# Oneflow-Inc/libai

Measured on AMD Instinct MI355X. Metric: tokens/sec (whole node), GPT-2 345M 3D-parallel at 1/2/4/8 MI355X, higher is better.
Workload: dtype bf16; 1 GPU; model=gpt2-345m (nl24 h1024 nah16 seq1024), global_batch=48, seq_len=1024, parallelism=dp1

## Files before the change

### libai_amd/csrc/kernels/adamw.hip

```cpp
#include "common.h"
#include "launchers.h"

namespace {

constexpr int CHUNK = 1 << 16;

struct AdamChunkDesc {
  int64_t param;
  int64_t master;
  int64_t grad;
  int64_t m;
  int64_t v;
  int64_t n;
};

template <class E>
__global__ void adamw_kernel(const AdamChunkDesc* __restrict__ chunks, float lr,
                             float beta1, float beta2, float eps, float wd,
                             float bc1, float bc2,
                             float grad_scale) {
  const AdamChunkDesc c = chunks[blockIdx.x];
  const int64_t n = c.n;
  typename E::T* p16 = (typename E::T*)c.param;
  float* master = (float*)c.master;
  const typename E::T* g = (const typename E::T*)c.grad;
  float* m = (float*)c.m;
  float* v = (float*)c.v;
  const float inv_bc1 = 1.0f / bc1, inv_bc2 = 1.0f / bc2;

  for (int64_t i = threadIdx.x; i < n; i += blockDim.x) {
    float gv = E::to_f(g[i]) * grad_scale;
    float pv = master[i];
    float mv = m[i] = beta1 * m[i] + (1.0f - beta1) * gv;
    float vv = v[i] = beta2 * v[i] + (1.0f - beta2) * gv * gv;
    float mhat = mv * inv_bc1;
    float vhat = vv * inv_bc2;
    pv -= lr * (mhat / (sqrtf(vhat) + eps) + wd * pv);
    master[i] = pv;
    if (p16) p16[i] = E::from_f(pv);
  }
}

struct NormChunkDesc {
  int64_t ptr;
  int64_t n;
};

template <class E>
__global__ void l2norm_sq_kernel(const NormChunkDesc* __restrict__ chunks,
                                 float* __restrict__ out) {
  __shared__ float red[16];
  const NormChunkDesc c = chunks[blockIdx.x];
  const typename E::T* x = (const typename E::T*)c.ptr;
  float s = 0.f;
  for (int64_t i = threadIdx.x; i < c.n; i += blockDim.x) {
    float v = E::to_f(x[i]);
    s += v * v;
  }
  s = block_reduce(s, red, SumOp(), 0.f);
  if (threadIdx.x == 0) atomicAdd(out, s);
}

}

extern "C" int adamw_chunk_elems() { return CHUNK; }

#define ADAMW_LAUNCHERS(SUFF, ETYPE)                                                   \
  extern "C" void adamw_step_##SUFF(const void* chunks, int nchunks, float lr,         \
                                    float beta1, float beta2, float eps, float wd,     \
                                    float bc1, float bc2, float grad_scale,            \
                                    hipStream_t stream) {                              \
    adamw_kernel<ETYPE><<<dim3(nchunks), dim3(256), 0, stream>>>(                      \
        (const AdamChunkDesc*)chunks, lr, beta1, beta2, eps, wd, bc1, bc2,             \
        grad_scale);                                                                   \
  }                                                                                    \
  extern "C" void l2norm_sq_##SUFF(const void* chunks, int nchunks, float* out,        \
                                   hipStream_t stream) {                               \
    l2norm_sq_kernel<ETYPE><<<dim3(nchunks), dim3(256), 0, stream>>>(                  \
        (const NormChunkDesc*)chunks, out);                                            \
  }

ADAMW_LAUNCHERS(bf16, BF16Elem)
ADAMW_LAUNCHERS(f32, F32Elem)
```

### libai_amd/csrc/kernels/common.h

```cpp
#pragma once
#include <hip/hip_runtime.h>
#include <stdint.h>

#include <type_traits>

#define WAVE 64

__device__ __forceinline__ float bf2f(uint16_t h) {
  union {
    uint32_t u;
    float f;
  } v;
  v.u = ((uint32_t)h) << 16;
  return v.f;
}

__device__ __forceinline__ uint16_t f2bf(float f) {
  union {
    float f;
    uint32_t u;
  } v;
  v.f = f;
  uint32_t lsb = (v.u >> 16) & 1u;
  uint32_t rounded = v.u + 0x7fffu + lsb;
  if ((v.u & 0x7f800000u) == 0x7f800000u) rounded = v.u;
  return (uint16_t)(rounded >> 16);
}

typedef uint16_t u16x8 __attribute__((ext_vector_type(8)));
typedef uint16_t u16x4 __attribute__((ext_vector_type(4)));
typedef float f32x4 __attribute__((ext_vector_type(4)));

struct BF16Elem {
  using T = uint16_t;
  static constexpr int VEC = 8;
  using VecT = u16x8;
  static __device__ __forceinline__ float to_f(T x) { return bf2f(x); }
  static __device__ __forceinline__ T from_f(float x) { return f2bf(x); }
};

struct F32Elem {
  using T = float;
  static constexpr int VEC = 4;
  using VecT = f32x4;
  static __device__ __forceinline__ float to_f(T x) { return x; }
  static __device__ __forceinline__ T from_f(float x) { return x; }
};

__device__ __forceinline__ float wave_reduce_sum(float v) {
#pragma unroll
  for (int off = WAVE / 2; off > 0; off >>= 1) v += __shfl_xor(v, off, WAVE);
  return v;
}

__device__ __forceinline__ float wave_reduce_max(float v) {
#pragma unroll
  for (int off = WAVE / 2; off > 0; off >>= 1) v = fmaxf(v, __shfl_xor(v, off, WAVE));
  return v;
}

template <typename Op>
__device__ __forceinline__ float block_reduce(float v, float* lds, Op op, float ident) {
  const int lane = threadIdx.x & (WAVE - 1);
  const int wid = threadIdx.x / WAVE;
  const int nw = (blockDim.x + WAVE - 1) / WAVE;
#pragma unroll
  for (int off = WAVE / 2; off > 0; off >>= 1) v = op(v, __shfl_xor(v, off, WAVE));
  if (lane == 0) lds[wid] = v;
  __syncthreads();
  v = (threadIdx.x < nw) ? lds[threadIdx.x] : ident;
  if (wid == 0) {
#pragma unroll
    for (int off = WAVE / 2; off > 0; off >>= 1) v = op(v, __shfl_xor(v, off, WAVE));
    if (lane == 0) lds[0] = v;
  }
  __syncthreads();
  v = lds[0];
  __syncthreads();
  return v;
}

struct SumOp {
  __device__ float operator()(float a, float b) const { return a + b; }
};
struct MaxOp {
  __device__ float operator()(float a, float b) const { return fmaxf(a, b); }
};

__device__ __forceinline__ void philox_round(uint32_t& c0, uint32_t& c1, uint32_t& c2,
                                             uint32_t& c3, uint32_t k0, uint32_t k1) {
  const uint32_t M0 = 0xD2511F53u, M1 = 0xCD9E8D57u;
  uint32_t h0 = __umulhi(M0, c0), l0 = M0 * c0;
  uint32_t h1 = __umulhi(M1, c2), l1 = M1 * c2;
  uint32_t n0 = h1 ^ c1 ^ k0;
  uint32_t n1 = l1;
  uint32_t n2 = h0 ^ c3 ^ k1;
  uint32_t n3 = l0;
  c0 = n0;
  c1 = n1;
  c2 = n2;
  c3 = n3;
}

__device__ __forceinline__ void philox4(uint64_t seed, uint64_t ctr, uint32_t out[4]) {
  uint32_t k0 = (uint32_t)seed, k1 = (uint32_t)(seed >> 32);
  uint32_t c0 = (uint32_t)ctr, c1 = (uint32_t)(ctr >> 32), c2 = 0x9E3779B9u, c3 = 0xBB67AE85u;
#pragma unroll
  for (int i = 0; i < 10; ++i) {
    philox_round(c0, c1, c2, c3, k0, k1);
    k0 += 0x9E3779B9u;
    k1 += 0xBB67AE85u;
  }
  out[0] = c0;
  out[1] = c1;
  out[2] = c2;
  out[3] = c3;
}

__device__ __forceinline__ float u32_to_uniform(uint32_t x) {
  return (x >> 8) * (1.0f / 16777216.0f);
}

#define RND_HASH_LO_MUL 0x9E3779B9u
#define RND_HASH_HI_MUL 0x85EBCA6Bu

__device__ __forceinline__ uint32_t rnd_hash_mix(uint32_t h) {
  h ^= h >> 16;
  h *= 0x7FEB352Du;
  h ^= h >> 15;
  h *= 0x846CA68Bu;
  h ^= h >> 16;
  return h;
}

__device__ __forceinline__ uint32_t rnd_hash2(uint64_t seed, uint32_t lo,
                                               uint32_t hi) {
  return rnd_hash_mix((uint32_t)seed ^ (lo * RND_HASH_LO_MUL) ^
                      (hi * RND_HASH_HI_MUL) ^ (uint32_t)(seed >> 32));
}

__device__ __forceinline__ uint32_t rnd_hash(uint64_t seed, uint64_t idx) {
  return rnd_hash2(seed, (uint32_t)idx, (uint32_t)(idx >> 32));
}

__device__ __forceinline__ uint32_t drop_threshold_u8(float p) {
  float t = p * 256.0f + 0.5f;
  return t >= 255.f ? 255u : (uint32_t)t;
}

__device__ __forceinline__ uint32_t drop_threshold_u32(float p) {
  double t = (double)p * 4294967296.0;
  return (t >= 4294967295.0) ? 0xFFFFFFFFu : (uint32_t)t;
}

__device__ __forceinline__ float fast_erff(float x) {
  const float a1 = 0.254829592f, a2 = -0.284496736f, a3 = 1.421413741f;
  const float a4 = -1.453152027f, a5 = 1.061405429f, p = 0.3275911f;
  float ax = fabsf(x);
  float t = 1.0f / fmaf(p, ax, 1.0f);
  float poly = t * fmaf(t, fmaf(t, fmaf(t, fmaf(t, a5, a4), a3), a2), a1);
  float y = 1.0f - poly * __expf(-ax * ax);
  return copysignf(y, x);
}

__device__ __forceinline__ float gelu_erf(float x) {
  return 0.5f * x * (1.0f + fast_erff(x * 0.70710678118654752440f));
}

__device__ __forceinline__ float gelu_erf_grad(float x) {
  const float kInvSqrt2 = 0.70710678118654752440f;
  const float kInvSqrt2Pi = 0.3989422804014327f;
  float cdf = 0.5f * (1.0f + fast_erff(x * kInvSqrt2));
  float pdf = kInvSqrt2Pi * __expf(-0.5f * x * x);
  return cdf + x * pdf;
}

#define CDIV(a, b) (((a) + (b)-1) / (b))

enum class FlashVariant : int { kPlain, kAlibi, kWindow, kRelBias, kDocs };

inline FlashVariant flash_variant(const float* alibi_slopes, int window,
                                  const float* rel_bias, const int* doc_start) {
  if (alibi_slopes != nullptr) return FlashVariant::kAlibi;
  if (window > 0) return FlashVariant::kWindow;
  if (rel_bias != nullptr) return FlashVariant::kRelBias;
  if (doc_start != nullptr) return FlashVariant::kDocs;
  return FlashVariant::kPlain;
}

template <class F>
void flash_dispatch(int D, FlashVariant v, F&& f) {
  auto on_d = [&](auto d) {
#define FLASH_VARIANT_CASE(NAME)                                             \
  case FlashVariant::NAME:                                                   \
    f(d, std::integral_constant<FlashVariant, FlashVariant::NAME>{});        \
    break;
    switch (v) {
      FLASH_VARIANT_CASE(kPlain)
      FLASH_VARIANT_CASE(kAlibi)
      FLASH_VARIANT_CASE(kWindow)
      FLASH_VARIANT_CASE(kRelBias)
      FLASH_VARIANT_CASE(kDocs)
    }
#undef FLASH_VARIANT_CASE
  };
  if (D == 64) on_d(std::integral_constant<int, 64>{});
  else if (D == 128) on_d(std::integral_constant<int, 128>{});
}
```

### libai_amd/csrc/kernels/fused_bias.hip

```cpp
#include "common.h"
#include "launchers.h"

namespace {

template <class E, bool GRAD>
__global__ void bias_gelu_kernel(const typename E::T* __restrict__ x,
                                 const typename E::T* __restrict__ b,
                                 const typename E::T* __restrict__ dy,
                                 typename E::T* __restrict__ out,
                                 float* __restrict__ db_partial, int64_t n,
                                 int W) {
  using VecT = typename E::VecT;
  constexpr int V = E::VEC;
  const int wvec = W / V;
  const int64_t R = n / W;
  const int cv = blockIdx.x * blockDim.x + threadIdx.x;
  if (cv >= wvec) return;
  VecT vb;
  if (b) vb = ((const VecT*)b)[cv];
  float db[GRAD ? V : 1] = {0.f};
  for (int64_t r = blockIdx.y; r < R; r += gridDim.y) {
    const int64_t i = r * wvec + cv;
    VecT vx = ((const VecT*)x)[i];
    VecT o;
    if (GRAD) {
      VecT vdy = ((const VecT*)dy)[i];
#pragma unroll
      for (int j = 0; j < V; ++j) {
        float xv = E::to_f(vx[j]) + (b ? E::to_f(vb[j]) : 0.f);
        float g = E::to_f(vdy[j]) * gelu_erf_grad(xv);
        o[j] = E::from_f(g);
        db[j] += g;
      }
    } else {
#pragma unroll
      for (int j = 0; j < V; ++j) {
        float xv = E::to_f(vx[j]) + (b ? E::to_f(vb[j]) : 0.f);
        o[j] = E::from_f(gelu_erf(xv));
      }
    }
    ((VecT*)out)[i] = o;
  }
  if (GRAD && db_partial != nullptr) {
#pragma unroll
    for (int j = 0; j < V; ++j)
      db_partial[(int64_t)blockIdx.y * W + cv * V + j] = db[j];
  }
}

template <class E, bool GRAD>
__global__ void bias_dropout_res_kernel(const typename E::T* __restrict__ x,
                                        const typename E::T* __restrict__ b,
                                        const typename E::T* __restrict__ res,
                                        typename E::T* __restrict__ out,
                                        float* __restrict__ db_partial, int64_t n,
                                        int W, float p, uint64_t seed) {
  using VecT = typename E::VecT;
  constexpr int V = E::VEC;
  const int wvec = W / V;
  const int64_t R = n / W;
  const float scale = 1.0f / (1.0f - p);
  const uint32_t thr8 = drop_threshold_u8(p);
  const int cv = blockIdx.x * blockDim.x + threadIdx.x;
  if (cv >= wvec) return;
  VecT vb;
  if (b) vb = ((const VecT*)b)[cv];
  float db[GRAD ? V : 1] = {0.f};
  for (int64_t r = blockIdx.y; r < R; r += gridDim.y) {
    const int64_t i = r * wvec + cv;
    VecT vx = ((const VecT*)x)[i];
    float keep[V];
    if (p > 0.f) {
#pragma unroll
      for (int q = 0; q < V / 4; ++q) {
        const uint64_t idx = (uint64_t)i * (V / 4) + q;
        const uint32_t h = rnd_hash(seed, idx);
#pragma unroll
        for (int j = 0; j < 4; ++j)
          keep[q * 4 + j] = (((h >> (j * 8)) & 0xFFu) >= thr8) ? scale : 0.f;
      }
    } else {
#pragma unroll
      for (int j = 0; j < V; ++j) keep[j] = 1.f;
    }
    VecT o;
    if (GRAD) {
#pragma unroll
      for (int j = 0; j < V; ++j) {
        float g = E::to_f(vx[j]) * keep[j];
        o[j] = E::from_f(g);
        db[j] += g;
      }
    } else {
      VecT vr;
      if (res) vr = ((const VecT*)res)[i];
#pragma unroll
      for (int j = 0; j < V; ++j) {
        float v = (E::to_f(vx[j]) + (b ? E::to_f(vb[j]) : 0.f)) * keep[j];
        o[j] = E::from_f(v + (res ? E::to_f(vr[j]) : 0.f));
      }
    }
    ((VecT*)out)[i] = o;
  }
  if (GRAD && db_partial != nullptr) {
#pragma unroll
    for (int j = 0; j < V; ++j)
      db_partial[(int64_t)blockIdx.y * W + cv * V + j] = db[j];
  }
}

template <class E>
__global__ void colsum_partial_kernel(const typename E::T* __restrict__ in,
                                      float* __restrict__ partial, int64_t R, int W) {
  using VecT = typename E::VecT;
  constexpr int V = E::VEC;
  const int wv = W / V;
  const int jv = blockIdx.x * blockDim.x + threadIdx.x;
  if (jv >= wv) return;
  const int P = gridDim.y;
  float s[V];
#pragma unroll
  for (int j = 0; j < V; ++j) s[j] = 0.f;
  for (int64_t r = blockIdx.y; r < R; r += P) {
    VecT v = ((const VecT*)(in + r * W))[jv];
#pragma unroll
    for (int j = 0; j < V; ++j) s[j] += E::to_f(v[j]);
  }
#pragma unroll
  for (int j = 0; j < V; ++j) partial[(int64_t)blockIdx.y * W + jv * V + j] = s[j];
}

template <class E>
__global__ void colsum_partial_scalar_kernel(const typename E::T* __restrict__ in,
                                             float* __restrict__ partial, int64_t R,
                                             int W) {
  const int j = blockIdx.x * blockDim.x + threadIdx.x;
  if (j >= W) return;
  const int P = gridDim.y;
  float s = 0.f;
  for (int64_t r = blockIdx.y; r < R; r += P) s += E::to_f(in[r * W + j]);
  partial[(int64_t)blockIdx.y * W + j] = s;
}

inline int64_t ew_grid(int64_t nvec) {
  int64_t g = CDIV(nvec, 256);
  return g < 2048 ? g : 2048;
}

inline dim3 col_grid(int64_t n, int W, int V, int* block_out) {
  const int wvec = W / V;
  const int block = wvec < 256 ? wvec : 256;
  const int gx = (int)CDIV(wvec, block);
  int64_t rows = n / W;
  int64_t gy = 4096 / gx;
  if (gy > rows) gy = rows;
  if (gy < 1) gy = 1;
  *block_out = block;
  return dim3(gx, (uint32_t)gy);
}

}

extern "C" int bias_col_grid_rows(int64_t n, int W, int V) {
  int blk;
  dim3 g = col_grid(n, W, V, &blk);
  return (int)g.y;
}

#define BIAS_LAUNCHERS(SUFF, ETYPE)                                                      \
  extern "C" void bias_gelu_fwd_##SUFF(const void* x, const void* b, void* y, int64_t n, \
                                       int W, hipStream_t stream) {                      \
    int blk;                                                                             \
    dim3 g = col_grid(n, W, ETYPE::VEC, &blk);                                           \
    bias_gelu_kernel<ETYPE, false><<<g, dim3(blk), 0, stream>>>(                         \
        (const ETYPE::T*)x, (const ETYPE::T*)b, nullptr, (ETYPE::T*)y, nullptr, n,       \
        W);                                                                              \
  }                                                                                      \
  extern "C" void bias_gelu_bwd_##SUFF(const void* x, const void* b, const void* dy,     \
                                       void* dx, float* db_partial, int64_t n, int W,    \
                                       hipStream_t stream) {                             \
    int blk;                                                                             \
    dim3 g = col_grid(n, W, ETYPE::VEC, &blk);                                           \
    bias_gelu_kernel<ETYPE, true><<<g, dim3(blk), 0, stream>>>(                          \
        (const ETYPE::T*)x, (const ETYPE::T*)b, (const ETYPE::T*)dy, (ETYPE::T*)dx,      \
        db_partial, n, W);                                                               \
  }                                                                                      \
  extern "C" void bias_dropout_res_fwd_##SUFF(const void* x, const void* b,              \
                                              const void* res, void* y, int64_t n,       \
                                              int W, float p, uint64_t seed,             \
                                              hipStream_t stream) {                      \
    int blk;                                                                             \
    dim3 g = col_grid(n, W, ETYPE::VEC, &blk);                                           \
    bias_dropout_res_kernel<ETYPE, false><<<g, dim3(blk), 0, stream>>>(                  \
        (const ETYPE::T*)x, (const ETYPE::T*)b, (const ETYPE::T*)res, (ETYPE::T*)y,      \
        nullptr, n, W, p, seed);                                                         \
  }                                                                                      \
  extern "C" void bias_dropout_res_bwd_##SUFF(const void* dy, void* dx,                  \
                                              float* db_partial, int64_t n, int W,       \
                                              float p, uint64_t seed,                    \
                                              hipStream_t stream) {                      \
    int blk;                                                                             \
    dim3 g = col_grid(n, W, ETYPE::VEC, &blk);                                           \
    bias_dropout_res_kernel<ETYPE, true><<<g, dim3(blk), 0, stream>>>(                   \
        (const ETYPE::T*)dy, nullptr, nullptr, (ETYPE::T*)dx, db_partial, n, W, p,       \
        seed);                                                                           \
  }                                                                                      \
  extern "C" void colsum_##SUFF(const void* in, float* partial, void* out, int64_t R,    \
                                int W, int P, hipStream_t stream) {                      \
    if (W % ETYPE::VEC == 0)                                                             \
      colsum_partial_kernel<ETYPE>                                                       \
          <<<dim3(CDIV(W / ETYPE::VEC, 256), P), dim3(256), 0, stream>>>(                \
              (const ETYPE::T*)in, partial, R, W);                                       \
    else                                                                                 \
      colsum_partial_scalar_kernel<ETYPE>                                                \
          <<<dim3(CDIV(W, 256), P), dim3(256), 0, stream>>>(                             \
              (const ETYPE::T*)in, partial, R, W);                                       \
    (void)out;                                                                           \
  }

BIAS_LAUNCHERS(bf16, BF16Elem)
BIAS_LAUNCHERS(f32, F32Elem)
```

Baseline: 297,500 tokens/s.

## Vectorize AdamW and L2-norm kernels, use hardware bf16 convert and fast erf reciprocal

Rewrites the AdamW kernel to process eight elements per thread with 16-byte vector loads and stores, falling back to a scalar tail when pointers are misaligned. It also vectorizes the grad-norm reduction. It replaces the manual float-to-bf16 rounding with a builtin cast and swaps the erf division for a refined hardware reciprocal. The bias-GeLU kernel is restructured and uses explicit FMA control, which changes numerics slightly (including per-lane fused vs unfused paths) in exchange for cheaper elementwise work.

Result: faster. 302,100 tokens/s (median of 6 runs) (+1.6%).

```diff
diff --git a/libai_amd/csrc/kernels/adamw.hip b/libai_amd/csrc/kernels/adamw.hip
--- a/libai_amd/csrc/kernels/adamw.hip
+++ b/libai_amd/csrc/kernels/adamw.hip
@@ -14,11 +14,38 @@
   int64_t n;
 };
 
+struct AdamHyper {
+  float lr, beta1, beta2, eps, wd, inv_bc1, inv_bc2, grad_scale;
+  float omb1, omb2;
+};
+
+template <class E>
+__device__ __forceinline__ void adamw_elem(float g, float& p, float& m, float& v,
+                                           const AdamHyper& h) {
+#pragma clang fp contract(off)
+  const float gv = g * h.grad_scale;
+  const float t = h.omb2 * gv;
+  if constexpr (std::is_same<E, BF16Elem>::value) {
+    m = fmaf(h.beta1, m, h.omb1 * gv);
+    v = fmaf(h.beta2, v, gv * t);
+  } else {
+    m = fmaf(h.omb1, gv, h.beta1 * m);
+    v = fmaf(gv, t, h.beta2 * v);
+  }
+  const float mhat = m * h.inv_bc1;
+  const float vhat = v * h.inv_bc2;
+  p = fmaf(-h.lr, fmaf(h.wd, p, mhat / (sqrtf(vhat) + h.eps)), p);
+}
+
+constexpr int AVEC = 8;
+
 template <class E>
 __global__ void adamw_kernel(const AdamChunkDesc* __restrict__ chunks, float lr,
                              float beta1, float beta2, float eps, float wd,
                              float bc1, float bc2,
                              float grad_scale) {
+  using VecT = typename E::VecT;
+  constexpr int GV = AVEC / E::VEC;
   const AdamChunkDesc c = chunks[blockIdx.x];
   const int64_t n = c.n;
   typename E::T* p16 = (typename E::T*)c.param;
@@ -26,16 +53,52 @@
   const typename E::T* g = (const typename E::T*)c.grad;
   float* m = (float*)c.m;
   float* v = (float*)c.v;
-  const float inv_bc1 = 1.0f / bc1, inv_bc2 = 1.0f / bc2;
+  const AdamHyper h = {lr,          beta1,       beta2,      eps,
+                       wd,          1.0f / bc1,  1.0f / bc2, grad_scale,
+                       1.0f - beta1, 1.0f - beta2};
 
-  for (int64_t i = threadIdx.x; i < n; i += blockDim.x) {
-    float gv = E::to_f(g[i]) * grad_scale;
-    float pv = master[i];
-    float mv = m[i] = beta1 * m[i] + (1.0f - beta1) * gv;
-    float vv = v[i] = beta2 * v[i] + (1.0f - beta2) * gv * gv;
-    float mhat = mv * inv_bc1;
-    float vhat = vv * inv_bc2;
-    pv -= lr * (mhat / (sqrtf(vhat) + eps) + wd * pv);
+  const bool aligned = ((c.param | c.master | c.grad | c.m | c.v) & 15) == 0;
+  const int64_t nvec = aligned ? n - n % AVEC : 0;
+
+  for (int64_t i = (int64_t)threadIdx.x * AVEC; i < nvec;
+       i += (int64_t)blockDim.x * AVEC) {
+    VecT vg[GV];
+    f32x4 vp[2], vm[2], vv[2];
+#pragma unroll
+    for (int k = 0; k < GV; ++k) vg[k] = ((const VecT*)(g + i))[k];
+#pragma unroll
+    for (int k = 0; k < 2; ++k) {
+      vp[k] = ((const f32x4*)(master + i))[k];
+      vm[k] = ((const f32x4*)(m + i))[k];
+      vv[k] = ((const f32x4*)(v + i))[k];
+    }
+    VecT o[GV];
+#pragma unroll
+    for (int j = 0; j < AVEC; ++j) {
+      float pv = vp[j / 4][j % 4], mv = vm[j / 4][j % 4], sv = vv[j / 4][j % 4];
+      adamw_elem<E>(E::to_f(vg[j / E::VEC][j % E::VEC]), pv, mv, sv, h);
+      vp[j / 4][j % 4] = pv;
+      vm[j / 4][j % 4] = mv;
+      vv[j / 4][j % 4] = sv;
+      o[j / E::VEC][j % E::VEC] = E::from_f(pv);
+    }
+#pragma unroll
+    for (int k = 0; k < 2; ++k) {
+      ((f32x4*)(m + i))[k] = vm[k];
+      ((f32x4*)(v + i))[k] = vv[k];
+      ((f32x4*)(master + i))[k] = vp[k];
+    }
+    if (p16) {
+#pragma unroll
+      for (int k = 0; k < GV; ++k) ((VecT*)(p16 + i))[k] = o[k];
+    }
+  }
+
+  for (int64_t i = nvec + threadIdx.x; i < n; i += blockDim.x) {
+    float pv = master[i], mv = m[i], sv = v[i];
+    adamw_elem<E>(E::to_f(g[i]), pv, mv, sv, h);
+    m[i] = mv;
+    v[i] = sv;
     master[i] = pv;
     if (p16) p16[i] = E::from_f(pv);
   }
@@ -52,8 +115,20 @@
   __shared__ float red[16];
   const NormChunkDesc c = chunks[blockIdx.x];
   const typename E::T* x = (const typename E::T*)c.ptr;
+  using VecT = typename E::VecT;
+  constexpr int V = E::VEC;
   float s = 0.f;
-  for (int64_t i = threadIdx.x; i < c.n; i += blockDim.x) {
+  const int64_t nvec = (c.ptr & 15) == 0 ? c.n - c.n % V : 0;
+#pragma unroll 4
+  for (int64_t i = (int64_t)threadIdx.x * V; i < nvec; i += (int64_t)blockDim.x * V) {
+    const VecT vx = *(const VecT*)(x + i);
+#pragma unroll
+    for (int j = 0; j < V; ++j) {
+      float v = E::to_f(vx[j]);
+      s += v * v;
+    }
+  }
+  for (int64_t i = nvec + threadIdx.x; i < c.n; i += blockDim.x) {
     float v = E::to_f(x[i]);
     s += v * v;
   }
diff --git a/libai_amd/csrc/kernels/common.h b/libai_amd/csrc/kernels/common.h
--- a/libai_amd/csrc/kernels/common.h
+++ b/libai_amd/csrc/kernels/common.h
@@ -16,15 +16,7 @@
 }
 
 __device__ __forceinline__ uint16_t f2bf(float f) {
-  union {
-    float f;
-    uint32_t u;
-  } v;
-  v.f = f;
-  uint32_t lsb = (v.u >> 16) & 1u;
-  uint32_t rounded = v.u + 0x7fffu + lsb;
-  if ((v.u & 0x7f800000u) == 0x7f800000u) rounded = v.u;
-  return (uint16_t)(rounded >> 16);
+  return __builtin_bit_cast(uint16_t, (__bf16)f);
 }
 
 typedef uint16_t u16x8 __attribute__((ext_vector_type(8)));
@@ -153,26 +145,39 @@
   return (t >= 4294967295.0) ? 0xFFFFFFFFu : (uint32_t)t;
 }
 
+
+__device__ __forceinline__ float rcp_ge1(float d) {
+#pragma clang fp contract(off)
+  float r = __builtin_amdgcn_rcpf(d);
+  r = fmaf(fmaf(-d, r, 1.0f), r, r);
+  float q = r;
+  q = fmaf(fmaf(-d, q, 1.0f), r, q);
+  return fmaf(fmaf(-d, q, 1.0f), r, q);
+}
+
 __device__ __forceinline__ float fast_erff(float x) {
+#pragma clang fp contract(off)
   const float a1 = 0.254829592f, a2 = -0.284496736f, a3 = 1.421413741f;
   const float a4 = -1.453152027f, a5 = 1.061405429f, p = 0.3275911f;
   float ax = fabsf(x);
-  float t = 1.0f / fmaf(p, ax, 1.0f);
+  float t = rcp_ge1(fminf(fmaf(p, ax, 1.0f), 0x1p+96f));
   float poly = t * fmaf(t, fmaf(t, fmaf(t, fmaf(t, a5, a4), a3), a2), a1);
-  float y = 1.0f - poly * __expf(-ax * ax);
+  float y = fmaf(-__expf(-ax * ax), poly, 1.0f);
   return copysignf(y, x);
 }
 
 __device__ __forceinline__ float gelu_erf(float x) {
+#pragma clang fp contract(off)
   return 0.5f * x * (1.0f + fast_erff(x * 0.70710678118654752440f));
 }
 
-__device__ __forceinline__ float gelu_erf_grad(float x) {
+__device__ __forceinline__ float gelu_erf_grad(float x, bool fused = true) {
+#pragma clang fp contract(off)
   const float kInvSqrt2 = 0.70710678118654752440f;
   const float kInvSqrt2Pi = 0.3989422804014327f;
   float cdf = 0.5f * (1.0f + fast_erff(x * kInvSqrt2));
   float pdf = kInvSqrt2Pi * __expf(-0.5f * x * x);
-  return cdf + x * pdf;
+  return fused ? fmaf(x, pdf, cdf) : cdf + x * pdf;
 }
 
 #define CDIV(a, b) (((a) + (b)-1) / (b))
diff --git a/libai_amd/csrc/kernels/fused_bias.hip b/libai_amd/csrc/kernels/fused_bias.hip
--- a/libai_amd/csrc/kernels/fused_bias.hip
+++ b/libai_amd/csrc/kernels/fused_bias.hip
@@ -2,6 +2,30 @@
 #include "launchers.h"
 
 namespace {
+
+
+template <class E, bool GRAD>
+__device__ __forceinline__ typename E::VecT bias_gelu_vec(typename E::VecT vx,
+                                                          typename E::VecT vdy,
+                                                          const float* fb,
+                                                          float* db) {
+#pragma clang fp contract(off)
+  constexpr int V = E::VEC;
+  typename E::VecT o;
+#pragma unroll
+  for (int j = 0; j < V; ++j) {
+    const float xv = E::to_f(vx[j]) + fb[j];
+    if (GRAD) {
+      const float d = gelu_erf_grad(xv, j < V - 2);
+      const float dyv = E::to_f(vdy[j]);
+      o[j] = E::from_f(dyv * d);
+      db[j] = fmaf(d, dyv, db[j]);
+    } else {
+      o[j] = E::from_f(gelu_erf(xv));
+    }
+  }
+  return o;
+}
 
 template <class E, bool GRAD>
 __global__ void bias_gelu_kernel(const typename E::T* __restrict__ x,
@@ -16,30 +40,25 @@
   const int64_t R = n / W;
   const int cv = blockIdx.x * blockDim.x + threadIdx.x;
   if (cv >= wvec) return;
-  VecT vb;
-  if (b) vb = ((const VecT*)b)[cv];
+  float fb[V];
+  {
+    VecT vb;
+    if (b) vb = ((const VecT*)b)[cv];
+#pragma unroll
+    for (int j = 0; j < V; ++j) fb[j] = b ? E::to_f(vb[j]) : 0.f;
+  }
   float db[GRAD ? V : 1] = {0.f};
+  const VecT* xp = (const VecT*)x + cv;
+  VecT* op = (VecT*)out + cv;
+  auto load_dy = [&](int64_t i) {
+    VecT d = {};
+    if constexpr (GRAD) d = ((const VecT*)dy)[i + cv];
+    return d;
+  };
   for (int64_t r = blockIdx.y; r < R; r += gridDim.y) {
-    const int64_t i = r * wvec + cv;
-    VecT vx = ((const VecT*)x)[i];
-    VecT o;
-    if (GRAD) {
-      VecT vdy = ((const VecT*)dy)[i];
-#pragma unroll
-      for (int j = 0; j < V; ++j) {
-        float xv = E::to_f(vx[j]) + (b ? E::to_f(vb[j]) : 0.f);
-        float g = E::to_f(vdy[j]) * gelu_erf_grad(xv);
-        o[j] = E::from_f(g);
-        db[j] += g;
-      }
-    } else {
-#pragma unroll
-      for (int j = 0; j < V; ++j) {
-        float xv = E::to_f(vx[j]) + (b ? E::to_f(vb[j]) : 0.f);
-        o[j] = E::from_f(gelu_erf(xv));
-      }
-    }
-    ((VecT*)out)[i] = o;
+    const int64_t i = r * wvec;
+    const VecT vx = xp[i];
+    op[i] = bias_gelu_vec<E, GRAD>(vx, load_dy(i), fb, db);
   }
   if (GRAD && db_partial != nullptr) {
 #pragma unroll
```
